# lambdaclass/simpleworks

Hardware: AMD Instinct MI355X
Metric: Marlin prove() constraints/sec at 2^20 R1CS; G1 MSM points/sec (higher is better)
Workload: dtype u32 limbs (384-bit Montgomery Fq for G1, 256-bit Fr); 1 GPU; marlin_prove: synthetic R1CS, 2^20 constraints = variables = non-zeros per matrix (|H| = |K| = 2^20), SRS + proving key device resident; per_gpu_units=1048576, multi_gpu=replicas (one proof per rank)

## Files before the change

### include/swmarlin.h

```cpp
#ifndef SWMARLIN_H
#define SWMARLIN_H
#include <stddef.h>
#include <stdint.h>
#ifdef __cplusplus
extern "C" {
#endif

#define SWM_OK 0
#define SWM_ERR_INVALID_ARG (-1)
#define SWM_ERR_NO_DEVICE (-2)
#define SWM_ERR_HIP (-3)
#define SWM_ERR_OOM (-4)
#define SWM_ERR_UNSATISFIED (-5)
#define SWM_ERR_INDEX_TOO_LARGE (-6)
#define SWM_ERR_SERIALIZATION (-7)
#define SWM_ERR_MISMATCH (-8)
#define SWM_ERR_INTERNAL (-9)

typedef struct swm_ctx swm_ctx;
typedef struct swm_bases swm_bases;

int swm_version(void);
const char *swm_strerror(int code);
int swm_init(int device, swm_ctx **out);
// ... 108 lines not shown

typedef struct swm_pedersen swm_pedersen;
int swm_pedersen_create(swm_ctx *ctx, const uint8_t *generators_xy, size_t num_windows, size_t window_size, swm_pedersen **out);
void swm_pedersen_destroy(swm_ctx *ctx, swm_pedersen *params);
int swm_pedersen_hash(swm_ctx *ctx, const swm_pedersen *params, const uint8_t *inputs, size_t input_len, size_t count,
                      uint8_t *digests);
int swm_pedersen_hash_dev(swm_ctx *ctx, const swm_pedersen *params, const void *d_inputs, size_t input_len, size_t count,
                          void *d_digests);
int swm_merkle_tree_build(swm_ctx *ctx, const swm_pedersen *leaf_params, const swm_pedersen *two_to_one_params,
                          const uint8_t *leaves, size_t leaf_len, size_t n_leaves, uint8_t *nodes);
int swm_merkle_tree_build_dev(swm_ctx *ctx, const swm_pedersen *leaf_params, const swm_pedersen *two_to_one_params,
                              const void *d_leaves, size_t leaf_len, size_t n_leaves, void *d_nodes);

typedef int (*swm_allgather_fn)(void *user, const void *send, size_t bytes, void *recv);
int swm_set_msm_sharding(swm_ctx *ctx, unsigned rank, unsigned world, swm_allgather_fn allgather, void *user);

int swm_rccl_unique_id(uint8_t out[128]);
int swm_rccl_init(swm_ctx *ctx, const uint8_t id[128], unsigned rank, unsigned world);
int swm_set_rccl_comm(swm_ctx *ctx, void *nccl_comm, unsigned rank, unsigned world);
int swm_exchange_stats(swm_ctx *ctx, uint64_t *calls, uint64_t *bytes_per_rank);
int swm_rccl_info(char *buf, size_t cap);

int swm_profile_enable(swm_ctx *ctx, int on);
int swm_device_mem_info(swm_ctx *ctx, size_t *free_bytes, size_t *total_bytes);
int swm_profile_reset(swm_ctx *ctx);
int swm_profile_json(swm_ctx *ctx, char *buf, size_t buflen);

int swm_selftest_exchange(swm_ctx *ctx, const void *d_send, void *d_recv, size_t bytes_per_peer, int alltoall);
int swm_selftest_mul(swm_ctx *ctx, int which, const uint64_t *a, const uint64_t *b, uint64_t *out, size_t n);
int swm_selftest_g1_add(swm_ctx *ctx, const uint64_t *a_xy, const uint64_t *b_xy, uint64_t *out_jac, size_t n);
int swm_selftest_g1_codec(swm_ctx *ctx, int op, const void *in, size_t n, void *out, unsigned *bad);
int swm_selftest_mul_throughput(swm_ctx *ctx, int which, size_t threads, int iters, float *ms);
int swm_selftest_pairing(unsigned *failed);
int swm_selftest_fr_inv(const uint64_t *a_mont, uint64_t *out_mont, size_t n, unsigned *fallbacks);
int swm_selftest_fr29(swm_ctx *ctx, int op, const uint32_t *a9, const uint32_t *b9, const uint32_t *spread9, uint32_t *out9,
                      size_t n);
int swm_selftest_poly(swm_ctx *ctx, int op, void *data, size_t n, size_t m, const uint64_t z[4], const uint64_t *pieces,
                      size_t npieces, void *out);
int swm_selftest_sample_fr(swm_ctx *ctx, swm_rng *rng, size_t need, uint64_t *out_mont);
int swm_selftest_verify_batch(swm_ctx *ctx, const swm_vk *vk, const uint64_t *public_inputs, size_t n_inputs,
                              const uint8_t *const *proofs, const size_t *lens, size_t count, unsigned flags, swm_rng *rng,
                              int *ok, int *results, uint64_t tw_xy[12], uint64_t tc_xy[12]);

#ifdef __cplusplus
}
#endif
#endif
```

### simpleworks_amd/_lib.py

```python
import ctypes
import json
import os

import numpy as np

_HERE = os.path.dirname(os.path.abspath(__file__))
LIB_PATH = os.environ.get("SWM_LIB_PATH") or os.path.join(_HERE, "libswmarlin.so")

_u64p = ctypes.POINTER(ctypes.c_uint64)
_u32p = ctypes.POINTER(ctypes.c_uint32)
_vp = ctypes.c_void_p
_sz = ctypes.c_size_t
_int = ctypes.c_int

ABI = {
    "swm_version": (_int, []),
    "swm_strerror": (ctypes.c_char_p, [_int]),
    "swm_init": (_int, [_int, ctypes.POINTER(_vp)]),
    "swm_destroy": (None, [_vp]),
    "swm_last_error": (ctypes.c_char_p, [_vp]),
    "swm_set_stream": (_int, [_vp, _vp]),
    "swm_set_msm_sharding": (_int, [_vp, ctypes.c_uint, ctypes.c_uint, _vp, _vp]),
    "swm_rccl_unique_id": (_int, [ctypes.c_void_p]),
    "swm_rccl_init": (_int, [_vp, ctypes.c_void_p, ctypes.c_uint, ctypes.c_uint]),
# ... 46 lines not shown
    "swm_pk_refcount": (_int, [_vp]),
    "swm_device_mem_info": (_int, [_vp, ctypes.POINTER(_sz), ctypes.POINTER(_sz)]),
    "swm_vk_destroy": (None, [_vp]),
    "swm_generate_proof": (_int, [_vp, _vp, ctypes.c_void_p, _vp, ctypes.c_void_p, _sz, ctypes.POINTER(_sz)]),
    "swm_generate_proof_ex": (_int, [_vp, _vp, ctypes.c_void_p, _vp, ctypes.c_uint, ctypes.c_void_p, _sz, ctypes.POINTER(_sz)]),
    "swm_proof_recode": (_int, [ctypes.c_void_p, _sz, _int, ctypes.c_void_p, _sz, ctypes.POINTER(_sz)]),
    "swm_verify_proof": (_int, [_vp, _u64p, _sz, ctypes.c_void_p, _sz, _vp, ctypes.POINTER(_int)]),
    "swm_vk_serialize": (_int, [_vp, ctypes.c_void_p, _sz, ctypes.POINTER(_sz)]),
    "swm_vk_deserialize": (_int, [ctypes.c_void_p, _sz, ctypes.POINTER(_vp)]),
    "swm_proof_validate": (_int, [ctypes.c_void_p, _sz]),
    "swm_pk_serialize": (_int, [_vp, _vp, ctypes.c_void_p, _sz, ctypes.POINTER(_sz)]),
    "swm_pk_deserialize": (_int, [_vp, ctypes.c_void_p, _sz, ctypes.POINTER(_vp)]),
    "swm_pk_serialize_ex": (_int, [_vp, _vp, ctypes.c_uint, ctypes.c_void_p, _sz, ctypes.POINTER(_sz)]),
    "swm_pk_deserialize_ex": (_int, [_vp, ctypes.c_void_p, _sz, ctypes.c_uint, ctypes.POINTER(_vp)]),
    "swm_vk_serialize_ex": (_int, [_vp, ctypes.c_uint, ctypes.c_void_p, _sz, ctypes.POINTER(_sz)]),
    "swm_vk_deserialize_ex": (_int, [ctypes.c_void_p, _sz, ctypes.c_uint, ctypes.POINTER(_vp)]),
    "swm_r1cs_is_satisfied": (_int, [_vp, ctypes.c_void_p, ctypes.POINTER(_int), ctypes.POINTER(_sz)]),
    "swm_blake2s": (_int, [ctypes.c_void_p, _sz, ctypes.c_void_p]),
    "swm_chacha_block": (_int, [ctypes.c_void_p, ctypes.c_uint64, _int, ctypes.c_void_p]),
    "swm_pedersen_create": (_int, [_vp, ctypes.c_void_p, _sz, _sz, ctypes.POINTER(_vp)]),
    "swm_pedersen_destroy": (None, [_vp, _vp]),
    "swm_pedersen_hash": (_int, [_vp, _vp, ctypes.c_void_p, _sz, _sz, ctypes.c_void_p]),
    "swm_pedersen_hash_dev": (_int, [_vp, _vp, _vp, _sz, _sz, _vp]),
    "swm_merkle_tree_build": (_int, [_vp, _vp, _vp, ctypes.c_void_p, _sz, _sz, ctypes.c_void_p]),
    "swm_merkle_tree_build_dev": (_int, [_vp, _vp, _vp, _vp, _sz, _sz, _vp]),
    "swm_profile_enable": (_int, [_vp, _int]),
    "swm_profile_reset": (_int, [_vp]),
    "swm_profile_json": (_int, [_vp, ctypes.c_char_p, _sz]),
    "swm_selftest_mul": (_int, [_vp, _int, _u64p, _u64p, _u64p, _sz]),
    "swm_selftest_g1_add": (_int, [_vp, _u64p, _u64p, _u64p, _sz]),
    "swm_selftest_g1_codec": (_int, [_vp, _int, ctypes.c_void_p, _sz, ctypes.c_void_p, ctypes.POINTER(ctypes.c_uint)]),
    "swm_selftest_mul_throughput": (_int, [_vp, _int, _sz, _int, ctypes.POINTER(ctypes.c_float)]),
    "swm_selftest_pairing": (_int, [ctypes.POINTER(ctypes.c_uint)]),
    "swm_selftest_fr_inv": (_int, [_u64p, _u64p, _sz, ctypes.POINTER(ctypes.c_uint)]),
    "swm_selftest_fr29": (_int, [_vp, _int, _u32p, _u32p, _u32p, _u32p, _sz]),
    "swm_selftest_poly": (_int, [_vp, _int, ctypes.c_void_p, _sz, _sz, _u64p, _u64p, _sz, ctypes.c_void_p]),
    "swm_selftest_sample_fr": (_int, [_vp, _vp, _sz, _u64p]),
    "swm_verify_proofs_batch": (_int, [_vp, _vp, _u64p, _sz, _vp, ctypes.POINTER(_sz), _sz, ctypes.c_uint, _vp,
                                       ctypes.POINTER(_int), ctypes.POINTER(_int)]),
    "swm_selftest_verify_batch": (_int, [_vp, _vp, _u64p, _sz, _vp, ctypes.POINTER(_sz), _sz, ctypes.c_uint, _vp,
                                         ctypes.POINTER(_int), ctypes.POINTER(_int), _u64p, _u64p]),
}


def rccl_info():
    buf = ctypes.create_string_buffer(1024)
    rc = load_library().swm_rccl_info(buf, len(buf))
    return rc == 0, buf.value.decode(errors="replace")


def rccl_unique_id():
    buf = (ctypes.c_uint8 * 128)()
    rc = load_library().swm_rccl_unique_id(buf)
    if rc != 0:
        raise SwmError(rc, "swm_rccl_unique_id", load_library().swm_last_error(None).decode(errors="replace"))
    return bytes(buf)


class SwmError(RuntimeError):
    def __init__(self, code, what, detail=""):
        self.code = code
        super().__init__("%s failed: %s (%d)%s" % (what, _strerror(code), code, (": " + detail) if detail else ""))


_lib = None

# ... 190 lines not shown

    def ntt_fr_dev(self, dbuf, log_n, inverse=False, coset=False):
        ptr = dbuf.ptr if isinstance(dbuf, DeviceBuffer) else int(dbuf)
        self._check(self.lib.swm_ntt_fr_dev(self.h, ptr, log_n, int(inverse), int(coset)), "swm_ntt_fr_dev")

    def ntt_fr_sharded_dev(self, dbuf, log_n, inverse=False, blocks_in=False):
        ptr = dbuf.ptr if isinstance(dbuf, DeviceBuffer) else int(dbuf)
        self._check(self.lib.swm_ntt_fr_sharded_dev(self.h, ptr, log_n, int(inverse), int(blocks_in)), "swm_ntt_fr_sharded_dev")

    def spmv_fr(self, rowptr, col, val_mont, z_mont):
        rowptr = np.ascontiguousarray(rowptr, dtype=np.uint32)
        col = np.ascontiguousarray(col, dtype=np.uint32)
        val = np.ascontiguousarray(val_mont, dtype=np.uint64).reshape(-1, 4)
        z = np.ascontiguousarray(z_mont, dtype=np.uint64).reshape(-1, 4)
        rows = rowptr.shape[0] - 1
        out = np.zeros((rows, 4), dtype=np.uint64)
        self._check(self.lib.swm_spmv_fr(self.h, _p32(rowptr), _p32(col) if col.size else _p32(np.zeros(1, np.uint32)),
                                         _p64(val) if val.size else _p64(np.zeros(4, np.uint64)), _p64(z), z.shape[0],
                                         _p64(out), rows, col.shape[0]), "swm_spmv_fr")
        return out

    def spmv_fr_dev(self, d_rowptr, d_col, d_val, d_z, d_out, rows):
        self._check(self.lib.swm_spmv_fr_dev(self.h, d_rowptr.ptr, d_col.ptr, d_val.ptr, d_z.ptr, d_out.ptr, rows),
                    "swm_spmv_fr_dev")

    def batch_inverse_fr(self, data_mont):
        d = np.ascontiguousarray(data_mont, dtype=np.uint64).reshape(-1, 4).copy()
        self._check(self.lib.swm_batch_inverse_fr(self.h, _p64(d), d.shape[0]), "swm_batch_inverse_fr")
        return d

    def batch_inverse_fr_dev(self, dbuf, n):
        self._check(self.lib.swm_batch_inverse_fr_dev(self.h, dbuf.ptr, n), "swm_batch_inverse_fr_dev")

    def vec_mul_fr(self, a, b):
        a = np.ascontiguousarray(a, dtype=np.uint64).reshape(-1, 4)
        b = np.ascontiguousarray(b, dtype=np.uint64).reshape(-1, 4)
        out = np.empty_like(a)
        self._check(self.lib.swm_vec_mul_fr(self.h, _p64(a), _p64(b), _p64(out), a.shape[0]), "swm_vec_mul_fr")
        return out

    def pedersen_create(self, generators_xy, num_windows, window_size):
        buf = np.ascontiguousarray(np.frombuffer(bytes(generators_xy), dtype=np.uint8))
        assert buf.size == 64 * num_windows * window_size
        h = _vp()
        self._check(self.lib.swm_pedersen_create(self.h, buf.ctypes.data, num_windows, window_size, ctypes.byref(h)),
                    "swm_pedersen_create")
        return h

    def pedersen_destroy(self, handle):
        if self.h and handle:
            self.lib.swm_pedersen_destroy(self.h, handle)

    def pedersen_hash(self, handle, inputs):
        a = np.ascontiguousarray(inputs, dtype=np.uint8)
        assert a.ndim == 2
        out = np.empty((a.shape[0], 32), dtype=np.uint8)
        self._check(self.lib.swm_pedersen_hash(self.h, handle, a.ctypes.data, a.shape[1], a.shape[0], out.ctypes.data),
                    "swm_pedersen_hash")
        return out

    def merkle_tree_build(self, leaf_handle, two_to_one_handle, leaves):
        a = np.ascontiguousarray(leaves, dtype=np.uint8)
        assert a.ndim == 2
        out = np.empty((2 * a.shape[0] - 1, 32), dtype=np.uint8)
        self._check(self.lib.swm_merkle_tree_build(self.h, leaf_handle, two_to_one_handle, a.ctypes.data, a.shape[1], a.shape[0],
                                                   out.ctypes.data), "swm_merkle_tree_build")
# ... 130 lines not shown
```

### simpleworks_amd/csrc/capi.hip

```cpp
#include <dlfcn.h>
#include <stdarg.h>
#include <string.h>
#include <algorithm>
#include <vector>
#include "context.h"
#include "g1.cuh"
#include "msm.h"

struct swm_rccl_id_arg {
    char internal[128];
};

namespace swm {

int ntt_run(swm_ctx* ctx, void* d_data, unsigned log_n, int inverse, int coset);
int ntt_sharded_run(swm_ctx* ctx, void* d_local, unsigned log_n, int inverse, int blocks_in);
struct SpmvPlan;
int spmv_run(swm_ctx* ctx, const void* d_rowptr, const void* d_col, const void* d_val, const void* d_z, void* d_out,
             size_t rows, const SpmvPlan* plan = nullptr);
int vec_mul_run(swm_ctx* ctx, const void* a, const void* b, void* out, size_t n);
int batch_inverse_run(swm_ctx* ctx, void* d, size_t n);
int selftest_mul_run(swm_ctx* ctx, int which, const void* a, const void* b, void* out, size_t n);
int selftest_chain_run(swm_ctx* ctx, int which, void* out, size_t threads, int iters);
int selftest_g1_add_run(swm_ctx* ctx, const void* a, const void* b, void* out, size_t n);
// ... 697 lines not shown
    SWM_ON_DEVICE(ctx);
    return spmv_run(ctx, d_rowptr, d_col, d_val, d_z, d_out, rows);
}
int swm_spmv_fr(swm_ctx* ctx, const uint32_t* rowptr, const uint32_t* col, const uint64_t* val, const uint64_t* z,
                size_t z_len, uint64_t* out, size_t rows, size_t nnz) {
    if (!ctx || !rowptr || !out || (nnz && (!col || !val || !z)))
        return set_err(ctx, SWM_ERR_INVALID_ARG, "spmv: bad arguments");
    SWM_ON_DEVICE(ctx);
    if (rowptr[rows] != nnz) return set_err(ctx, SWM_ERR_INVALID_ARG, "spmv: rowptr[rows] != nnz");
    for (size_t k = 0; k < nnz; k++)
        if (col[k] >= z_len) return set_err(ctx, SWM_ERR_INVALID_ARG, "spmv: column index out of range");
    char* d = nullptr;
    size_t o_rowptr = 0, o_col = (rows + 1) * 4, o_val = o_col + nnz * 4;
    o_val = (o_val + 31) & ~(size_t)31;
    size_t o_z = o_val + nnz * 32, o_out = o_z + z_len * 32, total = o_out + rows * 32;
    SWM_TRY(scratch(ctx, "stage.spmv", total + 64, (void**)&d));
    SWM_HIP(ctx, hipMemcpyAsync(d + o_rowptr, rowptr, (rows + 1) * 4, hipMemcpyHostToDevice, ctx->stream));
    if (nnz) {
        SWM_HIP(ctx, hipMemcpyAsync(d + o_col, col, nnz * 4, hipMemcpyHostToDevice, ctx->stream));
        SWM_HIP(ctx, hipMemcpyAsync(d + o_val, val, nnz * 32, hipMemcpyHostToDevice, ctx->stream));
        SWM_HIP(ctx, hipMemcpyAsync(d + o_z, z, z_len * 32, hipMemcpyHostToDevice, ctx->stream));
    }
    SWM_TRY(spmv_run(ctx, d + o_rowptr, d + o_col, d + o_val, d + o_z, d + o_out, rows));
    SWM_HIP(ctx, hipMemcpyAsync(out, d + o_out, rows * 32, hipMemcpyDeviceToHost, ctx->stream));
    SWM_HIP(ctx, hipStreamSynchronize(ctx->stream));
    return SWM_OK;
}

int swm_batch_inverse_fr_dev(swm_ctx* ctx, void* d_data, size_t n) {
    if (!ctx || (n && !d_data)) return set_err(ctx, SWM_ERR_INVALID_ARG, "batch_inverse: bad arguments");
    SWM_ON_DEVICE(ctx);
    return batch_inverse_run(ctx, d_data, n);
}
int swm_batch_inverse_fr(swm_ctx* ctx, uint64_t* data, size_t n) {
    if (!ctx || (n && !data)) return set_err(ctx, SWM_ERR_INVALID_ARG, "batch_inverse: bad arguments");
    SWM_ON_DEVICE(ctx);
    void* d = nullptr;
    SWM_TRY(scratch(ctx, "stage.a", n * 32 + 32, &d));
    SWM_HIP(ctx, hipMemcpyAsync(d, data, n * 32, hipMemcpyHostToDevice, ctx->stream));
    SWM_TRY(batch_inverse_run(ctx, d, n));
    SWM_HIP(ctx, hipMemcpyAsync(data, d, n * 32, hipMemcpyDeviceToHost, ctx->stream));
    SWM_HIP(ctx, hipStreamSynchronize(ctx->stream));
    return SWM_OK;
}
int swm_vec_mul_fr_dev(swm_ctx* ctx, const void* a, const void* b, void* out, size_t n) {
    if (!ctx || (n && (!a || !b || !out))) return set_err(ctx, SWM_ERR_INVALID_ARG, "vec_mul: bad arguments");
    SWM_ON_DEVICE(ctx);
    return vec_mul_run(ctx, a, b, out, n);
}
int swm_vec_mul_fr(swm_ctx* ctx, const uint64_t* a, const uint64_t* b, uint64_t* out, size_t n) {
    if (!ctx || (n && (!a || !b || !out))) return set_err(ctx, SWM_ERR_INVALID_ARG, "vec_mul: bad arguments");
    SWM_ON_DEVICE(ctx);
    char *da = nullptr, *db = nullptr;
    SWM_TRY(scratch(ctx, "stage.a", n * 32 + 32, (void**)&da));
    SWM_TRY(scratch(ctx, "stage.b", n * 32 + 32, (void**)&db));
    SWM_HIP(ctx, hipMemcpyAsync(da, a, n * 32, hipMemcpyHostToDevice, ctx->stream));
    SWM_HIP(ctx, hipMemcpyAsync(db, b, n * 32, hipMemcpyHostToDevice, ctx->stream));
    SWM_TRY(vec_mul_run(ctx, da, db, da, n));
    SWM_HIP(ctx, hipMemcpyAsync(out, da, n * 32, hipMemcpyDeviceToHost, ctx->stream));
    SWM_HIP(ctx, hipStreamSynchronize(ctx->stream));
    return SWM_OK;
}

int swm_profile_enable(swm_ctx* ctx, int on) {
    if (!ctx) return SWM_ERR_INVALID_ARG;
    SWM_ON_DEVICE(ctx);
// ... 126 lines not shown
```

### simpleworks_amd/csrc/context.h

```cpp
#pragma once
#include <hip/hip_runtime.h>
#include <stdint.h>
#include <stdio.h>
#include <map>
#include <string>
#include <vector>
#include "../../include/swmarlin.h"
#include "host/pool.h"
#include "switches.h"

namespace swm {

struct MsmJob;
struct DevBuf {
    void* p = nullptr;
    size_t cap = 0;
};

struct NttTables {
    void* lo = nullptr;
    void* hi = nullptr;
    size_t hi_len = 0;
};

// ... 38 lines not shown
    swm::MsmJob* lazy_tail = nullptr;
    int next_slot = 0;
    std::multimap<size_t, void*> pool;
    uint64_t stat_msm_digits = 0;
    uint64_t stat_msm_twins = 0;
    uint64_t stat_msm_adds = 0;
    uint64_t stat_msm_zero_points = 0;
    uint64_t stat_spmv_nnz = 0;
    std::vector<std::pair<char, uint64_t>> call_log;
    void log_call(char kind, uint64_t v) {
        if (profiling && call_log.size() < 8192) call_log.push_back({kind, v});
    }
    uint64_t stat_msm_calls = 0, stat_msm_points = 0, stat_ntt_calls = 0, stat_ntt_elems = 0, stat_spmv_calls = 0,
             stat_spmv_rows = 0;
    int profiling = 0;
    bool prof_open = false;
    std::map<std::string, swm::ProfAgg> prof;
    std::vector<swm::ProfPending> pending;
    std::vector<hipEvent_t> event_pool;
    unsigned shard_rank = 0, shard_world = 1;
    swm_allgather_fn shard_allgather = nullptr;
    void* shard_user = nullptr;
    void* rccl_comm = nullptr;
    bool rccl_own = false;
    void *rccl_send = nullptr, *rccl_recv = nullptr;
    size_t rccl_cap = 0;
    uint64_t stat_exchanges = 0, stat_exchange_bytes = 0;
    swm::HostPool* host_pool = nullptr;
    hipStream_t copy_stream = nullptr;
    void* ext_pinned = nullptr;
    bool ext_registered = false;
    size_t msm_pipe_min = 0;
    size_t msm_slot_bytes[6] = {0, 0, 0, 0, 0, 0};
    bool emulated_exchange = false;
    unsigned msm_since_wait = 0;
    uint32_t* ext_totals = nullptr;
    hipEvent_t ext_cnt_event[8] = {nullptr, nullptr, nullptr, nullptr, nullptr, nullptr, nullptr, nullptr};
    hipEvent_t ext_event[5] = {nullptr, nullptr, nullptr, nullptr, nullptr};
};

struct swm_bases {
    void* d_points = nullptr;
    void* d_points28 = nullptr;
    uint32_t* d_inf_mask = nullptr;
    unsigned table_c = 0;
    void* d_te = nullptr;
    size_t n = 0;
};

namespace swm {

int set_err(swm_ctx* ctx, int code, const char* fmt, ...);
void drain_streams(swm_ctx* ctx);
int shard_exchange(swm_ctx* ctx, const void* send, size_t bytes, void* recv);
int shard_allgather_dev(swm_ctx* ctx, const void* d_send, size_t bytes, void* d_recv);
int shard_alltoall_dev(swm_ctx* ctx, const void* d_send, void* d_recv, size_t bytes_per_peer);

struct DeviceGuard {
    int prev = -1;
    bool ok = true, switched = false;
    explicit DeviceGuard(const swm_ctx* ctx) {
        if (!ctx) return;
        if (hipGetDevice(&prev) != hipSuccess) prev = -1;
        if (prev != ctx->device) {
            ok = hipSetDevice(ctx->device) == hipSuccess;
            switched = ok && prev >= 0;
// ... 42 lines not shown
```

### simpleworks_amd/csrc/marlin.hip

```cpp
#include <stdlib.h>
#include <string.h>
#include <algorithm>
#include <chrono>
#include <functional>
#include <memory>
#include "devops.cuh"
#include "g1.cuh"
#include "host/ahp.h"

#include "msm.h"
using namespace swm;

#define LAUNCHX(ctx, name, kernel, grid, block, shmem, ...)                         \
    do {                                                                            \
        prof_begin(ctx, name);                                                      \
        hipLaunchKernelGGL(kernel, grid, block, shmem, (ctx)->stream, __VA_ARGS__); \
        prof_end(ctx);                                                              \
        hip_check(ctx, hipGetLastError(), name);                                    \
    } while (0)

#include "host/pk_codec.h"
#include "host/host_handles.h"
struct swm_srs {
    ~swm_srs() {
        if (d_powers) (void)hipFree(d_powers);
    }
    size_t max_degree = 0;
    bool in_subgroup = false;
    G1Affine* d_powers = nullptr;
    std::vector<G1Affine> gamma_powers;
    G2Affine h, beta_h;
};

namespace {

struct DevCsr {
    DBuf<uint32_t> rowptr, col;
    DVec val;
    size_t rows = 0, nnz = 0;
// ... 1266 lines not shown
void r_alpha(swm_ctx* ctx, const swm_pk& pk, ProveState& s) {
    const Fr alpha = s.st.alpha;
    const uint64_t M = s.M;
    s.r_alpha_evals = DVec(ctx, s.H);
    {
        Fr a4h = alpha;
        for (unsigned i = 0; i < s.logM; i++) a4h = fp_sqr(a4h);
        s.ra_closed_form = !fp_is_one(a4h) && !sw(SW_RALPHA_TRANSFORMS);
    }
    if (!s.ra_closed_form) return r_alpha_on_h(ctx, pk, s);
    if (s.sp.r2) {
        const size_t mloc = s.sp.Mloc, mblk = s.sp.Mblk, s_rank = s.sp.rank;
        s.e_ra = DVec(ctx, mloc);
        PowTable wt = root_pow_table(ctx, s.logM);
        Fr* out = s.e_ra.p;
        ew(ctx, "r_alpha_den", mloc, [=] __device__(size_t p) {
            const size_t i = mloc * (p / mblk) + s_rank * mblk + (p % mblk);
            out[p] = fp_sub(alpha, wt.at(i));
        });
        rc_check(ctx, batch_inverse_run(ctx, out, mloc));
        const RAlphaNumerators nu = r_alpha_numerators(alpha, pk.logH, M);
        ew(ctx, "r_alpha_scale", mloc, [=] __device__(size_t p) {
            const size_t i = mloc * (p / mblk) + s_rank * mblk + (p % mblk);
            const unsigned q = (unsigned)(i & 3);
            out[p] = fp_mul(out[p], q == 0 ? nu.n0 : q == 1 ? nu.n1 : q == 2 ? nu.n2 : nu.n3);
        });
        r_alpha_on_h(ctx, pk, s);
    } else if (s.cosets) {
        const uint64_t H = s.H;
        const unsigned logH = pk.logH;
        s.e_ra = DVec(ctx, 3 * H);
        PowTable wt = root_pow_table(ctx, s.logM);
        Fr* out = s.e_ra.p;
        ew(ctx, "r_alpha_den", 3 * H, [=] __device__(size_t p) { out[p] = fp_sub(alpha, wt.at(((p & (H - 1)) << 2) + (p >> logH))); });
        rc_check(ctx, batch_inverse_run(ctx, out, 3 * H));
        const RAlphaNumerators nu = r_alpha_numerators(alpha, pk.logH, M);
        Fr* rh = s.r_alpha_evals.p;
        ew(ctx, "r_alpha_scale", 3 * H, [=] __device__(size_t p) {
            const size_t q = p >> logH;
            Fr v = fp_mul(out[p], q == 0 ? nu.n0 : q == 1 ? nu.n1 : nu.n2);
            out[p] = v;
            if (q == 0) rh[p] = v;
        });
    } else {
        s.e_ra = DVec(ctx, M);
        PowTable wt = root_pow_table(ctx, s.logM);
        Fr* out = s.e_ra.p;
        ew(ctx, "r_alpha_den", M, [=] __device__(size_t i) { out[i] = fp_sub(alpha, wt.at(i)); });
        rc_check(ctx, batch_inverse_run(ctx, out, M));
        const RAlphaNumerators nu = r_alpha_numerators(alpha, pk.logH, M);
        Fr* rh = s.r_alpha_evals.p;
        ew(ctx, "r_alpha_scale", M, [=] __device__(size_t i) {
            const unsigned q = (unsigned)(i & 3);
            Fr v = fp_mul(out[i], q == 0 ? nu.n0 : q == 1 ? nu.n1 : q == 2 ? nu.n2 : nu.n3);
            out[i] = v;
            if (q == 0) rh[i >> 2] = v;
        });
    }
}

void round2_t(swm_ctx* ctx, const swm_pk& pk, ProveState& s) {
    const uint64_t H = s.H, X = s.X;
    const size_t nvars = s.nvars;
    const Fr eta_a = s.st.eta_a, eta_b = s.st.eta_b, eta_c = s.st.eta_c;
    s.t_poly = dv_zeros(ctx, H);
    {
        DVec ta(ctx, nvars), tb(ctx, nvars), tc(ctx, nvars);
        const Fr* ra = s.r_alpha_evals.p;
        rc_check(ctx, spmv_run(ctx, pk.at.rowptr.p, pk.at.col.p, pk.at.val.p, ra, ta.p, nvars, &pk.at.plan));
        rc_check(ctx, spmv_run(ctx, pk.bt.rowptr.p, pk.bt.col.p, pk.bt.val.p, ra, tb.p, nvars, &pk.bt.plan));
        rc_check(ctx, spmv_run(ctx, pk.ct.rowptr.p, pk.ct.col.p, pk.ct.val.p, ra, tc.p, nvars, &pk.ct.plan));
        Fr* out = s.t_poly.p;
        const Fr *pa = ta.p, *pb = tb.p, *pc = tc.p;
        ew(ctx, "t_evals", nvars, [=] __device__(size_t c) {
            Fr v = fp_add(fp_add(fp_mul(eta_a, pa[c]), fp_mul(eta_b, pb[c])), fp_mul(eta_c, pc[c]));
            out[reindex_by_subdomain(H, X, c)] = v;
// ... 115 lines not shown
        if (i < Hl << lg) pg[i] = pa[r * 4 * Hl + 3 * Hl + j];
    });
}

void round2_commitments(swm_ctx* ctx, const swm_pk& pk, ProveState& s) {
    const uint64_t H = s.H;
    s.P_g1.p = s.g1x.p + 1; s.P_g1.n = H - 1; s.P_g1.has_bound = true; s.P_g1.bound = H - 2; s.P_g1.hiding = true;
    s.P_h1.p = s.h1.p; s.P_h1.n = 2 * H + 1;
    pc_commit_begin(ctx, pk, &s.lane, s.P_h1.p, s.P_h1.n, false, 0, false, &s.j2[2]);
    pc_commit_begin(ctx, pk, &s.lane, s.P_g1.p, s.P_g1.n, true, H - 2, true, &s.j2[1]);
    commit_flush(ctx);
    Fr rem0 = s.g1x.download(0, 1)[0];
    bool unsat = !fp_is_zero(rem0);
    pc_commit_blind(pk, &s.j2[0], nullptr, &s.P_t.rand);
    pc_commit_blind(pk, &s.j2[1], &s.zk, &s.P_g1.rand);
    pc_commit_blind(pk, &s.j2[2], nullptr, &s.P_h1.rand);
    commit_gather(ctx, {&s.j2[0].plain, &s.j2[1].plain, &s.j2[1].shifted, &s.j2[2].plain});
    pc_commit_end_round(ctx, pk, {&s.j2[0], &s.j2[1], &s.j2[2]}, {nullptr, &s.zk, nullptr},
                        {&s.P_t.rand, &s.P_g1.rand, &s.P_h1.rand}, s.comms2.data());
    if (unsat && !ctx->emulated_exchange)
        throw MarlinError(SWM_ERR_UNSATISFIED, "outer sumcheck does not hold: constraint system is not satisfied");
}

void round3_polys(swm_ctx* ctx, const swm_pk& pk, ProveState& s) {
    const uint64_t K = s.K, Bsz = s.Bsz;
    const Fr alpha = s.st.alpha, beta = s.st.beta;
    const Fr eta_a = s.st.eta_a, eta_b = s.st.eta_b, eta_c = s.st.eta_c;
    const Fr vhab = fp_mul(s.dh.vanishing(alpha), s.dh.vanishing(beta));
    s.f = DVec(ctx, K);
    const bool f_cosets = SWM_OUTER_COSETS && !s.sp.r3 && Bsz == 4 * K && K >= OUTER_COSETS_MIN_H;
    DVec f_K;
    {
        DVec inv(ctx, 3 * K);
        for (int m = 0; m < 3; m++) {
            Fr* out = inv.p + (size_t)m * K;
            const Fr *rk = pk.ar[m].row_K.p, *ck = pk.ar[m].col_K.p;
            ew(ctx, "round3_den_K", K, [=] __device__(size_t i) { out[i] = fp_mul(fp_sub(beta, rk[i]), fp_sub(alpha, ck[i])); });
        }
        rc_check(ctx, batch_inverse_run(ctx, inv.p, 3 * K));
        Fr* out = s.f.p;
        const Fr *ia = inv.p, *ib = inv.p + K, *ic = inv.p + 2 * K;
        const Fr *va = pk.ar[0].val_K.p, *vb = pk.ar[1].val_K.p, *vc = pk.ar[2].val_K.p;
        if (f_cosets) {
            f_K = DVec(ctx, K);
            out = f_K.p;
        }
        ew(ctx, "round3_f_K", K, [=] __device__(size_t i) {
            Fr t = fp_add(fp_add(fp_mul(fp_mul(eta_a, va[i]), ia[i]), fp_mul(fp_mul(eta_b, vb[i]), ib[i])),
                          fp_mul(fp_mul(eta_c, vc[i]), ic[i]));
            out[i] = fp_mul(vhab, t);
        });
        if (f_cosets) rc_check(ctx, ntt_run_from(ctx, s.f.p, pk.logK, 1, 0, f_K.p, K));
        else dv_ntt(ctx, s.f, pk.logK, true);
    }
    s.P_g2.p = s.f.p + 1; s.P_g2.n = K - 1; s.P_g2.has_bound = true; s.P_g2.bound = K - 2;
    pc_commit_begin(ctx, pk, &s.lane, s.P_g2.p, s.P_g2.n, true, K - 2, false, &s.j3[0]);
    s.h2 = DVec(ctx, 3 * K);
    const IndexOnB ix{pk.ar[0].row_B.p, pk.ar[0].col_B.p, pk.ar[0].row_col_B.p, pk.ar[0].val_B.p,
                      pk.ar[1].row_B.p, pk.ar[1].col_B.p, pk.ar[1].row_col_B.p, pk.ar[1].val_B.p,
                      pk.ar[2].row_B.p, pk.ar[2].col_B.p, pk.ar[2].row_col_B.p, pk.ar[2].val_B.p};
    const Round3Challenges ch{alpha, beta, fp_mul(beta, alpha), eta_a, eta_b, eta_c, vhab};
    if (s.sp.r3) {
        const size_t Bloc = Bsz / s.sp.SG, Bblk = Bloc / s.sp.SG, Kl = K / s.sp.SG, s_rank = s.sp.rank;
        DVec e_f = shard_evals(ctx, s.sp, s.f.p, K, pk.logB);
        DVec ab(ctx, Bloc);
        Fr* out = ab.p;
        const Fr* pf = e_f.p;
        ew(ctx, "round3_pointwise_B", Bloc, [=] __device__(size_t p) {
            const size_t i = Bloc * (p / Bblk) + s_rank * Bblk + (p % Bblk);
            out[p] = round3_a_minus_bf(ix, ch, i, pf[p]);
        });
        rc_check(ctx, ntt_sharded_run(ctx, ab.p, pk.logB, 1, 1));
// ... 1000 lines not shown
```

### simpleworks_amd/csrc/vec.hip

```cpp
#include <string.h>
#include "context.h"
#include "fq28.cuh"
#include "fr29.cuh"
#include "frinv.cuh"
#include "g1.cuh"

namespace swm {

__global__ void __launch_bounds__(256) vec_mul_kernel(const Fr* __restrict__ a, const Fr* __restrict__ b,
                                                      Fr* __restrict__ out, size_t n) {
    SWM_LIGHT_KERNEL();
    for (size_t i = blockIdx.x * (size_t)blockDim.x + threadIdx.x; i < n; i += (size_t)gridDim.x * blockDim.x)
        out[i] = fp_mul(a[i], b[i]);
}

static constexpr int BINV_CHUNK = 16, BINV_CHUNK_SMALL = 4;
static constexpr int BINV_THREADS = 256;
template <int BINV_CHUNK>
__global__ void __launch_bounds__(BINV_THREADS) batch_inverse_kernel29(Fr* __restrict__ v, size_t n) {
    SWM_LIGHT_KERNEL();
    __shared__ Fr sp[BINV_THREADS], ss[BINV_THREADS];
    __shared__ Fr s_inv;
    const unsigned tid = threadIdx.x;
    size_t t = blockIdx.x * (size_t)blockDim.x + tid;
    size_t lo = t * BINV_CHUNK;
    size_t hi = lo + BINV_CHUNK < n ? lo + BINV_CHUNK : n;
    Fr pref[BINV_CHUNK];
    Fr29 acc = fr29_unpack(fp_one<Fr>());
#pragma unroll
    for (int i = 0; i < BINV_CHUNK; i++) {
        pref[i] = fr29_pack(acc);
        if (lo + i < hi) {
            Fr x = v[lo + i];
            if (!fp_is_zero(x)) acc = fr29_mul_fenced(acc, fr29_unpack(x));
        }
    }
    const Fr accp = fr29_pack(acc);
    sp[tid] = accp;
    ss[tid] = accp;
    __syncthreads();
    for (unsigned d = 1; d < BINV_THREADS; d <<= 1) {
        const bool hp = tid >= d, hs = tid + d < BINV_THREADS;
        Fr a = hp ? sp[tid - d] : accp, b = hs ? ss[tid + d] : accp;
        Fr mp = sp[tid], ms = ss[tid];
        __syncthreads();
        if (hp) sp[tid] = fr29_pack(fr29_mul_fenced(fr29_unpack(mp), fr29_unpack(a)));
        if (hs) ss[tid] = fr29_pack(fr29_mul_fenced(fr29_unpack(ms), fr29_unpack(b)));
        __syncthreads();
    }
    if (tid == 0) s_inv = fr_inv_single(fr29_pack(fr29_canonical(fr29_unpack(ss[0]), true)));
    __syncthreads();
    Fr29 inv = fr29_unpack(s_inv);
    if (tid > 0) inv = fr29_mul_fenced(inv, fr29_unpack(sp[tid - 1]));
    if (tid + 1 < BINV_THREADS) inv = fr29_mul_fenced(inv, fr29_unpack(ss[tid + 1]));
#pragma unroll
    for (int i = BINV_CHUNK - 1; i >= 0; i--) {
        if (lo + i < hi) {
            Fr x = v[lo + i];
            if (!fp_is_zero(x)) {
                v[lo + i] = fr29_pack(fr29_canonical(fr29_mul_fenced(inv, fr29_unpack(pref[i])), true));
                inv = fr29_mul_fenced(inv, fr29_unpack(x));
            }
        }
    }
}

int vec_mul_run(swm_ctx* ctx, const void* a, const void* b, void* out, size_t n) {
    if (n == 0) return SWM_OK;
    unsigned grid = (unsigned)std::min<size_t>((n + 255) / 256, 256 * 32);
    SWM_LAUNCH(ctx, "vec_mul", vec_mul_kernel, dim3(grid), dim3(256), 0, (const Fr*)a, (const Fr*)b, (Fr*)out, n);
    return SWM_OK;
}
int batch_inverse_run(swm_ctx* ctx, void* d, size_t n) {
    if (n == 0) return SWM_OK;
    static constexpr size_t small_below = 262144;
    if (n <= small_below) {
        const size_t threads = (n + BINV_CHUNK_SMALL - 1) / BINV_CHUNK_SMALL;
        const dim3 grid((unsigned)((threads + BINV_THREADS - 1) / BINV_THREADS));
        SWM_LAUNCH(ctx, "batch_inverse", batch_inverse_kernel29<BINV_CHUNK_SMALL>, grid, dim3(BINV_THREADS), 0, (Fr*)d, n);
        return SWM_OK;
    }
    const size_t threads = (n + BINV_CHUNK - 1) / BINV_CHUNK;
    const dim3 grid((unsigned)((threads + BINV_THREADS - 1) / BINV_THREADS));
    SWM_LAUNCH(ctx, "batch_inverse", batch_inverse_kernel29<BINV_CHUNK>, grid, dim3(BINV_THREADS), 0, (Fr*)d, n);
    return SWM_OK;
}

template <class F>
__global__ void __launch_bounds__(256) selftest_mul_kernel(const F* a, const F* b, F* out, size_t n) {
    size_t i = blockIdx.x * (size_t)blockDim.x + threadIdx.x;
    if (i < n) out[i] = fp_mul(a[i], b[i]);
}
template <class F>
__global__ void __launch_bounds__(256) selftest_mul_chain(F* out, int iters) {
    size_t i = blockIdx.x * (size_t)blockDim.x + threadIdx.x;
    F a = fp_one<F>(), b = fp_one<F>();
    a.v[0] ^= (uint32_t)i;
    b.v[1] ^= (uint32_t)(i * 2654435761u);
    for (int k = 0; k < iters; k++) {
        a = fp_mul(a, b);
        b = fp_mul(b, a);
    }
    out[i] = fp_add(a, b);
}
__global__ void __launch_bounds__(256) selftest_mul28_kernel(const Fq* a, const Fq* b, Fq* out, size_t n) {
    size_t i = blockIdx.x * (size_t)blockDim.x + threadIdx.x;
    if (i < n) out[i] = fq28_pack(fq28_canonical(fq28_mul(fq28_unpack(a[i]), fq28_unpack(b[i]))));
}
__global__ void __launch_bounds__(256) selftest_sqr28_kernel(const Fq* a, const Fq* b, Fq* out, size_t n) {
    size_t i = blockIdx.x * (size_t)blockDim.x + threadIdx.x;
    if (i < n) out[i] = fq28_pack(fq28_canonical(fq28_sqr(fq28_add(fq28_unpack(a[i]), fq28_unpack(b[i])))));
}
__global__ void __launch_bounds__(256) selftest_mul2_28_kernel(const Fq* a, const Fq* b, Fq* out, size_t n) {
    size_t i = blockIdx.x * (size_t)blockDim.x + threadIdx.x;
    if (i >= n) return;
    Fq28 ua = fq28_unpack(a[i]), ub = fq28_unpack(b[i]), x, y, c;
#pragma unroll
    for (int k = 0; k < 14; k++) {
// ... 149 lines not shown
```

Before: 22.74 million constraints/s.

## Fuse denominator generation and scaling into batch inverse kernel

```diff
diff --git a/include/swmarlin.h b/include/swmarlin.h
--- a/include/swmarlin.h
+++ b/include/swmarlin.h
@@ -164,6 +164,7 @@
 int swm_selftest_g1_codec(swm_ctx *ctx, int op, const void *in, size_t n, void *out, unsigned *bad);
 int swm_selftest_mul_throughput(swm_ctx *ctx, int which, size_t threads, int iters, float *ms);
 int swm_selftest_pairing(unsigned *failed);
+int swm_selftest_batch_inverse_tiles(swm_ctx *ctx, unsigned tiles);
 int swm_selftest_fr_inv(const uint64_t *a_mont, uint64_t *out_mont, size_t n, unsigned *fallbacks);
 int swm_selftest_fr29(swm_ctx *ctx, int op, const uint32_t *a9, const uint32_t *b9, const uint32_t *spread9, uint32_t *out9,
                       size_t n);
diff --git a/simpleworks_amd/_lib.py b/simpleworks_amd/_lib.py
--- a/simpleworks_amd/_lib.py
+++ b/simpleworks_amd/_lib.py
@@ -102,6 +102,7 @@
     "swm_selftest_g1_codec": (_int, [_vp, _int, ctypes.c_void_p, _sz, ctypes.c_void_p, ctypes.POINTER(ctypes.c_uint)]),
     "swm_selftest_mul_throughput": (_int, [_vp, _int, _sz, _int, ctypes.POINTER(ctypes.c_float)]),
     "swm_selftest_pairing": (_int, [ctypes.POINTER(ctypes.c_uint)]),
+    "swm_selftest_batch_inverse_tiles": (_int, [_vp, ctypes.c_uint]),
     "swm_selftest_fr_inv": (_int, [_u64p, _u64p, _sz, ctypes.POINTER(ctypes.c_uint)]),
     "swm_selftest_fr29": (_int, [_vp, _int, _u32p, _u32p, _u32p, _u32p, _sz]),
     "swm_selftest_poly": (_int, [_vp, _int, ctypes.c_void_p, _sz, _sz, _u64p, _u64p, _sz, ctypes.c_void_p]),
@@ -358,6 +359,9 @@
     def batch_inverse_fr_dev(self, dbuf, n):
         self._check(self.lib.swm_batch_inverse_fr_dev(self.h, dbuf.ptr, n), "swm_batch_inverse_fr_dev")
 
+    def selftest_batch_inverse_tiles(self, tiles):
+        self._check(self.lib.swm_selftest_batch_inverse_tiles(self.h, tiles), "swm_selftest_batch_inverse_tiles")
+
     def vec_mul_fr(self, a, b):
         a = np.ascontiguousarray(a, dtype=np.uint64).reshape(-1, 4)
         b = np.ascontiguousarray(b, dtype=np.uint64).reshape(-1, 4)
diff --git a/simpleworks_amd/csrc/binv.cuh b/simpleworks_amd/csrc/binv.cuh
--- /dev/null
+++ b/simpleworks_amd/csrc/binv.cuh
@@ -0,0 +1,176 @@
+#pragma once
+#include <algorithm>
+#include <atomic>
+#include "context.h"
+#include "fr29.cuh"
+#include "frinv.cuh"
+
+namespace swm {
+
+static constexpr int BINV_CHUNK = 16, BINV_CHUNK_SMALL = 4;
+static constexpr int BINV_THREADS = 256;
+static constexpr unsigned BINV_MAX_TILES = 16;
+template <int CHUNK, bool FUSED, class Load, class Store>
+__global__ void __launch_bounds__(BINV_THREADS, 2) batch_inverse_kernel29(Fr* v, size_t n, unsigned tiles, Load load, Store store) {
+    SWM_LIGHT_KERNEL();
+    __shared__ Fr sp[BINV_THREADS], ss[BINV_THREADS];
+    __shared__ Fr s_tot[BINV_MAX_TILES], s_tinv[BINV_MAX_TILES];
+    __shared__ Fr s_inv;
+    constexpr size_t TILE = (size_t)BINV_THREADS * CHUNK;
+    const unsigned tid = threadIdx.x;
+    const size_t base = (size_t)blockIdx.x * tiles * TILE;
+    if (base >= n) return;
+    const size_t tiles_left = (n - base + TILE - 1) / TILE;
+    const unsigned my_tiles = tiles_left < tiles ? (unsigned)tiles_left : tiles;
+    const bool ranged = my_tiles > 1;
+    if (ranged) {
+        for (unsigned j = 0; j < my_tiles; j++) {
+            const size_t lo = base + j * TILE + (size_t)tid * CHUNK;
+            Fr29 acc = fr29_unpack(fp_one<Fr>());
+#pragma unroll 1
+            for (int i = 0; i < CHUNK; i++) {
+                if (lo + i < n) {
+                    Fr x;
+                    if (FUSED) {
+                        x = load(lo + i);
+                        v[lo + i] = x;
+                    } else {
+                        x = v[lo + i];
+                    }
+                    if (!fp_is_zero(x)) acc = fr29_mul_fenced(acc, fr29_unpack(x));
+                }
+            }
+            sp[tid] = fr29_pack(acc);
+            __syncthreads();
+            for (unsigned d = BINV_THREADS / 2; d > 0; d >>= 1) {
+                if (tid < d) sp[tid] = fr29_pack(fr29_mul_fenced(fr29_unpack(sp[tid]), fr29_unpack(sp[tid + d])));
+                __syncthreads();
+            }
+            if (tid == 0) s_tot[j] = sp[0];
+        }
+        __syncthreads();
+        if (tid == 0) {
+            Fr29 all = fr29_unpack(s_tot[0]);
+            for (unsigned j = 1; j < my_tiles; j++) all = fr29_mul_fenced(all, fr29_unpack(s_tot[j]));
+            s_inv = fr_inv_single(fr29_pack(fr29_canonical(all, true)));
+        }
+        __syncthreads();
+        if (tid < my_tiles) {
+            Fr29 ti = fr29_unpack(s_inv);
+            for (unsigned j = 0; j < my_tiles; j++)
+                if (j != tid) ti = fr29_mul_fenced(ti, fr29_unpack(s_tot[j]));
+            s_tinv[tid] = fr29_pack(ti);
+        }
+        __syncthreads();
+    }
+    for (unsigned j = 0; j < my_tiles; j++) {
+        const size_t lo = base + j * TILE + (size_t)tid * CHUNK;
+        const size_t hi = lo + CHUNK < n ? lo + CHUNK : n;
+        if (FUSED && !ranged) {
+#pragma unroll 1
+            for (int i = 0; i < CHUNK; i++)
+                if (lo + i < hi) v[lo + i] = load(lo + i);
+        }
+        Fr pref[CHUNK];
+        Fr29 acc = fr29_unpack(fp_one<Fr>());
+#pragma unroll
+        for (int i = 0; i < CHUNK; i++) {
+            pref[i] = fr29_pack(acc);
+            if (lo + i < hi) {
+                Fr x = v[lo + i];
+                if (!fp_is_zero(x)) acc = fr29_mul_fenced(acc, fr29_unpack(x));
+            }
+        }
+        const Fr accp = fr29_pack(acc);
+        sp[tid] = accp;
+        ss[tid] = accp;
+        __syncthreads();
+        for (unsigned d = 1; d < BINV_THREADS; d <<= 1) {
+            const bool hp = tid >= d, hs = tid + d < BINV_THREADS;
+            Fr a = hp ? sp[tid - d] : accp, b = hs ? ss[tid + d] : accp;
+            Fr mp = sp[tid], ms = ss[tid];
+            __syncthreads();
+            if (hp) sp[tid] = fr29_pack(fr29_mul_fenced(fr29_unpack(mp), fr29_unpack(a)));
+            if (hs) ss[tid] = fr29_pack(fr29_mul_fenced(fr29_unpack(ms), fr29_unpack(b)));
+            __syncthreads();
+        }
+        if (tid == 0 && !ranged) s_inv = fr_inv_single(fr29_pack(fr29_canonical(fr29_unpack(ss[0]), true)));
+        __syncthreads();
+        Fr29 inv = fr29_unpack(ranged ? s_tinv[j] : s_inv);
+        if (tid > 0) inv = fr29_mul_fenced(inv, fr29_unpack(sp[tid - 1]));
+        if (tid + 1 < BINV_THREADS) inv = fr29_mul_fenced(inv, fr29_unpack(ss[tid + 1]));
+#pragma unroll
+        for (int i = CHUNK - 1; i >= 0; i--) {
+            if (lo + i < hi) {
+                Fr x = v[lo + i];
+                if (!fp_is_zero(x)) {
+                    store(lo + i, fr29_pack(fr29_canonical(fr29_mul_fenced(inv, fr29_unpack(pref[i])), true)));
+                    inv = fr29_mul_fenced(inv, fr29_unpack(x));
+                } else if (FUSED) {
+                    store(lo + i, x);
+                }
+            }
+        }
+        __syncthreads();
+    }
+}
+
+static constexpr size_t BINV_SMALL_BELOW = 262144;
+
+template <class K>
+inline unsigned binv_resident(swm_ctx* ctx, K kernel, std::atomic<unsigned>* cache) {
+    std::atomic<unsigned>& slot = cache[ctx->device & 63];
+    unsigned r = slot.load(std::memory_order_acquire);
+    if (!r) {
+        int per_cu = 0, cus = 0;
+        if (hipOccupancyMaxActiveBlocksPerMultiprocessor(&per_cu, kernel, BINV_THREADS, 0) != hipSuccess) per_cu = 0;
+        if (hipDeviceGetAttribute(&cus, hipDeviceAttributeMultiprocessorCount, ctx->device) != hipSuccess) cus = 0;
+        if (per_cu <= 0 || cus <= 0) (void)hipGetLastError();
+        r = (unsigned)std::max(1, per_cu) * (unsigned)std::max(1, cus);
+        slot.store(r, std::memory_order_release);
+    }
+    return r;
+}
+
+static constexpr bool BINV_RANGED_BY_OCCUPANCY = false;
+inline unsigned binv_tiles_for(size_t ntiles, unsigned resident) {
+    if (!BINV_RANGED_BY_OCCUPANCY) return 1;
+    return (unsigned)std::min<size_t>((ntiles + resident - 1) / resident, BINV_MAX_TILES);
+}
+
+template <bool FUSED, class Load, class Store>
+inline int batch_inverse_launch(swm_ctx* ctx, Fr* d, size_t n, Load load, Store store) {
+    if (n == 0) return SWM_OK;
+    const unsigned forced = ctx->binv_tiles;
+    if (!forced && n <= BINV_SMALL_BELOW) {
+        const size_t threads = (n + BINV_CHUNK_SMALL - 1) / BINV_CHUNK_SMALL;
+        const dim3 grid((unsigned)((threads + BINV_THREADS - 1) / BINV_THREADS));
+        SWM_LAUNCH(ctx, "batch_inverse", (batch_inverse_kernel29<BINV_CHUNK_SMALL, FUSED, Load, Store>), grid, dim3(BINV_THREADS), 0, d, n, 1u,
+                   load, store);
+        return SWM_OK;
+    }
+    const size_t ntiles = (n + (size_t)BINV_THREADS * BINV_CHUNK - 1) / ((size_t)BINV_THREADS * BINV_CHUNK);
+    unsigned tiles = forced;
+    if (!tiles) {
+        static std::atomic<unsigned> resident[64];
+        tiles = BINV_RANGED_BY_OCCUPANCY ? binv_tiles_for(ntiles, binv_resident(ctx, batch_inverse_kernel29<BINV_CHUNK, FUSED, Load, Store>, resident)) : 1;
+    }
+    tiles = std::min(std::max(tiles, 1u), BINV_MAX_TILES);
+    const dim3 grid((unsigned)((ntiles + tiles - 1) / tiles));
+    SWM_LAUNCH(ctx, "batch_inverse", (batch_inverse_kernel29<BINV_CHUNK, FUSED, Load, Store>), grid, dim3(BINV_THREADS), 0, d, n, tiles, load,
+               store);
+    return SWM_OK;
+}
+struct BinvStoreInPlace {
+    Fr* v;
+    __device__ __forceinline__ void operator()(size_t p, const Fr& inv) const { v[p] = inv; }
+};
+struct BinvNoLoad {
+    __device__ __forceinline__ Fr operator()(size_t) const { return fp_zero<Fr>(); }
+};
+template <class Load>
+inline int batch_inverse_of(swm_ctx* ctx, Fr* v, size_t n, Load load) {
+    return batch_inverse_launch<true>(ctx, v, n, load, BinvStoreInPlace{v});
+}
+
+}
diff --git a/simpleworks_amd/csrc/capi.hip b/simpleworks_amd/csrc/capi.hip
--- a/simpleworks_amd/csrc/capi.hip
+++ b/simpleworks_amd/csrc/capi.hip
@@ -753,6 +753,11 @@
     SWM_ON_DEVICE(ctx);
     return batch_inverse_run(ctx, d_data, n);
 }
+int swm_selftest_batch_inverse_tiles(swm_ctx* ctx, unsigned tiles) {
+    if (!ctx || tiles > 16) return set_err(ctx, SWM_ERR_INVALID_ARG, "batch_inverse_tiles: 0 (the library's rule) .. 16 tiles per workgroup");
+    ctx->binv_tiles = tiles;
+    return SWM_OK;
+}
 int swm_batch_inverse_fr(swm_ctx* ctx, uint64_t* data, size_t n) {
     if (!ctx || (n && !data)) return set_err(ctx, SWM_ERR_INVALID_ARG, "batch_inverse: bad arguments");
     SWM_ON_DEVICE(ctx);
diff --git a/simpleworks_amd/csrc/context.h b/simpleworks_amd/csrc/context.h
--- a/simpleworks_amd/csrc/context.h
+++ b/simpleworks_amd/csrc/context.h
@@ -94,6 +94,7 @@
     bool ext_registered = false;
     size_t msm_pipe_min = 0;
     size_t msm_slot_bytes[6] = {0, 0, 0, 0, 0, 0};
+    unsigned binv_tiles = 0;
     bool emulated_exchange = false;
     unsigned msm_since_wait = 0;
     uint32_t* ext_totals = nullptr;
diff --git a/simpleworks_amd/csrc/marlin.hip b/simpleworks_amd/csrc/marlin.hip
--- a/simpleworks_amd/csrc/marlin.hip
+++ b/simpleworks_amd/csrc/marlin.hip
@@ -5,6 +5,7 @@
 #include <functional>
 #include <memory>
 #include "devops.cuh"
+#include "binv.cuh"
 #include "g1.cuh"
 #include "host/ahp.h"
 
@@ -1337,16 +1338,18 @@
         s.e_ra = DVec(ctx, 3 * H);
         PowTable wt = root_pow_table(ctx, s.logM);
         Fr* out = s.e_ra.p;
-        ew(ctx, "r_alpha_den", 3 * H, [=] __device__(size_t p) { out[p] = fp_sub(alpha, wt.at(((p & (H - 1)) << 2) + (p >> logH))); });
-        rc_check(ctx, batch_inverse_run(ctx, out, 3 * H));
         const RAlphaNumerators nu = r_alpha_numerators(alpha, pk.logH, M);
-        Fr* rh = s.r_alpha_evals.p;
-        ew(ctx, "r_alpha_scale", 3 * H, [=] __device__(size_t p) {
-            const size_t q = p >> logH;
-            Fr v = fp_mul(out[p], q == 0 ? nu.n0 : q == 1 ? nu.n1 : nu.n2);
-            out[p] = v;
-            if (q == 0) rh[p] = v;
-        });
+        auto inv1 = [](const Fr& a) {
+            bool ok = false;
+            const Fr r = fr_inv_bingcd(a, &ok);
+            return ok ? r : fp_inv(a);
+        };
+        const Fr i0 = inv1(nu.n0), i1 = inv1(nu.n1), i2 = inv1(nu.n2);
+        rc_check(ctx, batch_inverse_of(ctx, out, 3 * H, [=] __device__(size_t p) {
+                     const size_t q = p >> logH;
+                     return fp_mul(fp_sub(alpha, wt.at(((p & (H - 1)) << 2) + q)), q == 0 ? i0 : q == 1 ? i1 : i2);
+                 }));
+        hip_check(ctx, hipMemcpyAsync(s.r_alpha_evals.p, out, H * sizeof(Fr), hipMemcpyDeviceToDevice, ctx->stream), "d2d");
     } else {
         s.e_ra = DVec(ctx, M);
         PowTable wt = root_pow_table(ctx, s.logM);
@@ -1528,12 +1531,16 @@
     DVec f_K;
     {
         DVec inv(ctx, 3 * K);
-        for (int m = 0; m < 3; m++) {
-            Fr* out = inv.p + (size_t)m * K;
-            const Fr *rk = pk.ar[m].row_K.p, *ck = pk.ar[m].col_K.p;
-            ew(ctx, "round3_den_K", K, [=] __device__(size_t i) { out[i] = fp_mul(fp_sub(beta, rk[i]), fp_sub(alpha, ck[i])); });
-        }
-        rc_check(ctx, batch_inverse_run(ctx, inv.p, 3 * K));
+        {
+            const Fr *rk0 = pk.ar[0].row_K.p, *ck0 = pk.ar[0].col_K.p, *rk1 = pk.ar[1].row_K.p, *ck1 = pk.ar[1].col_K.p;
+            const Fr *rk2 = pk.ar[2].row_K.p, *ck2 = pk.ar[2].col_K.p;
+            const unsigned logK = pk.logK;
+            rc_check(ctx, batch_inverse_of(ctx, inv.p, 3 * K, [=] __device__(size_t p) {
+                         const size_t m = p >> logK, i = p & (K - 1);
+                         const Fr *rk = m == 0 ? rk0 : m == 1 ? rk1 : rk2, *ck = m == 0 ? ck0 : m == 1 ? ck1 : ck2;
+                         return fp_mul(fp_sub(beta, rk[i]), fp_sub(alpha, ck[i]));
+                     }));
+        }
         Fr* out = s.f.p;
         const Fr *ia = inv.p, *ib = inv.p + K, *ic = inv.p + 2 * K;
         const Fr *va = pk.ar[0].val_K.p, *vb = pk.ar[1].val_K.p, *vc = pk.ar[2].val_K.p;
diff --git a/simpleworks_amd/csrc/vec.hip b/simpleworks_amd/csrc/vec.hip
--- a/simpleworks_amd/csrc/vec.hip
+++ b/simpleworks_amd/csrc/vec.hip
@@ -3,6 +3,7 @@
 #include "fq28.cuh"
 #include "fr29.cuh"
 #include "frinv.cuh"
+#include "binv.cuh"
 #include "g1.cuh"
 
 namespace swm {
@@ -14,57 +15,6 @@
         out[i] = fp_mul(a[i], b[i]);
 }
 
-static constexpr int BINV_CHUNK = 16, BINV_CHUNK_SMALL = 4;
-static constexpr int BINV_THREADS = 256;
-template <int BINV_CHUNK>
-__global__ void __launch_bounds__(BINV_THREADS) batch_inverse_kernel29(Fr* __restrict__ v, size_t n) {
-    SWM_LIGHT_KERNEL();
-    __shared__ Fr sp[BINV_THREADS], ss[BINV_THREADS];
-    __shared__ Fr s_inv;
-    const unsigned tid = threadIdx.x;
-    size_t t = blockIdx.x * (size_t)blockDim.x + tid;
-    size_t lo = t * BINV_CHUNK;
-    size_t hi = lo + BINV_CHUNK < n ? lo + BINV_CHUNK : n;
-    Fr pref[BINV_CHUNK];
-    Fr29 acc = fr29_unpack(fp_one<Fr>());
-#pragma unroll
-    for (int i = 0; i < BINV_CHUNK; i++) {
-        pref[i] = fr29_pack(acc);
-        if (lo + i < hi) {
-            Fr x = v[lo + i];
-            if (!fp_is_zero(x)) acc = fr29_mul_fenced(acc, fr29_unpack(x));
-        }
-    }
-    const Fr accp = fr29_pack(acc);
-    sp[tid] = accp;
-    ss[tid] = accp;
-    __syncthreads();
-    for (unsigned d = 1; d < BINV_THREADS; d <<= 1) {
-        const bool hp = tid >= d, hs = tid + d < BINV_THREADS;
-        Fr a = hp ? sp[tid - d] : accp, b = hs ? ss[tid + d] : accp;
-        Fr mp = sp[tid], ms = ss[tid];
-        __syncthreads();
-        if (hp) sp[tid] = fr29_pack(fr29_mul_fenced(fr29_unpack(mp), fr29_unpack(a)));
-        if (hs) ss[tid] = fr29_pack(fr29_mul_fenced(fr29_unpack(ms), fr29_unpack(b)));
-        __syncthreads();
-    }
-    if (tid == 0) s_inv = fr_inv_single(fr29_pack(fr29_canonical(fr29_unpack(ss[0]), true)));
-    __syncthreads();
-    Fr29 inv = fr29_unpack(s_inv);
-    if (tid > 0) inv = fr29_mul_fenced(inv, fr29_unpack(sp[tid - 1]));
-    if (tid + 1 < BINV_THREADS) inv = fr29_mul_fenced(inv, fr29_unpack(ss[tid + 1]));
-#pragma unroll
-    for (int i = BINV_CHUNK - 1; i >= 0; i--) {
-        if (lo + i < hi) {
-            Fr x = v[lo + i];
-            if (!fp_is_zero(x)) {
-                v[lo + i] = fr29_pack(fr29_canonical(fr29_mul_fenced(inv, fr29_unpack(pref[i])), true));
-                inv = fr29_mul_fenced(inv, fr29_unpack(x));
-            }
-        }
-    }
-}
-
 int vec_mul_run(swm_ctx* ctx, const void* a, const void* b, void* out, size_t n) {
     if (n == 0) return SWM_OK;
     unsigned grid = (unsigned)std::min<size_t>((n + 255) / 256, 256 * 32);
@@ -72,18 +22,7 @@
     return SWM_OK;
 }
 int batch_inverse_run(swm_ctx* ctx, void* d, size_t n) {
-    if (n == 0) return SWM_OK;
-    static constexpr size_t small_below = 262144;
-    if (n <= small_below) {
-        const size_t threads = (n + BINV_CHUNK_SMALL - 1) / BINV_CHUNK_SMALL;
-        const dim3 grid((unsigned)((threads + BINV_THREADS - 1) / BINV_THREADS));
-        SWM_LAUNCH(ctx, "batch_inverse", batch_inverse_kernel29<BINV_CHUNK_SMALL>, grid, dim3(BINV_THREADS), 0, (Fr*)d, n);
-        return SWM_OK;
-    }
-    const size_t threads = (n + BINV_CHUNK - 1) / BINV_CHUNK;
-    const dim3 grid((unsigned)((threads + BINV_THREADS - 1) / BINV_THREADS));
-    SWM_LAUNCH(ctx, "batch_inverse", batch_inverse_kernel29<BINV_CHUNK>, grid, dim3(BINV_THREADS), 0, (Fr*)d, n);
-    return SWM_OK;
+    return batch_inverse_launch<false>(ctx, (Fr*)d, n, BinvNoLoad{}, BinvStoreInPlace{(Fr*)d});
 }
 
 template <class F>
```

New measurement: 22.71 million constraints/s. Within noise of the previous version (-0.1%).
